# raulmur/ORB_SLAM2

Hardware: AMD Instinct MI355X
Metric: frames/s ORB extract+match, 1241x376 gray, 2000 kpts, 8 lvls (higher is better)
Workload: dtype u8

## Files before the change

### orb_slam2_amd/csrc/orbhip_api.hip

```cpp
#include <cstdarg>
#include <unistd.h>
#include <sys/syscall.h>
#include "orbhip_ctx.h"

static thread_local std::string g_err;
orbhip_status orbhip_set_error(orbhip_status st, const char* fmt, ...)
{
    char buf[512]; va_list ap; va_start(ap, fmt); vsnprintf(buf, sizeof buf, fmt, ap); va_end(ap);
    g_err = buf; return st;
}

static const char* kKernelNames[K_COUNT] = {"k_pyramid_level", "k_fast_cells", "k_blur", "k_quadtree", "k_describe",
                                            "k_match_grid", "k_match_candidates", "k_match_select", "k_undistort_keys", "k_remap"};

static const signed char kPatternHost[256 * 4] = {
#include "brief_pattern_31.inc"
};

void prof_collect(orbhip_ctx* c)
{
    for (auto& s : c->pending) {
        (void)hipEventSynchronize(s.b);
        float ms = 0; (void)hipEventElapsedTime(&ms, s.a, s.b);
        c->tot_ms[s.k] += ms; c->launches[s.k] += s.counts;
// ... 422 lines not shown
        std::vector<unsigned> mask(8 * 64, 0u);
        for (int q = 0; q < 8; q++) for (int l = 0; l < 64; l++) for (int b = 0; b < 4; b++) {
            const int r = 4 * q + (l >> 4), d = l & 15, v = r - 15, uu = 4 * d + b - 15;
            if (r <= 30 && d <= 7 && abs(uu) <= 15 && abs(uu) <= umax[abs(v)]) mask[q * 64 + l] |= 0xffu << (8 * b);
        }
        TRY(upload(&c->d_ic_mask, mask));
    }
    {
        const int psd = fc_pstride(c) / 4, nd = psd * std::max(c->fc_maxph, 1);
        c->fc_np = (nd + 63) / 64;
        const int np8 = (c->fc_np + 7) & ~7;
        std::vector<int4> tab((size_t)(np8 / 4) * 2 * 64);
        for (int k = 0; k < np8; k++) for (int l = 0; l < 64; l++) {
            const int pos = 64 * k + l, row = pos / psd, col4 = 4 * (pos % psd);
            int* r = &tab[(size_t)((k >> 2) * 2) * 64 + l].x; int* d = &tab[(size_t)((k >> 2) * 2 + 1) * 64 + l].x;
            r[k & 3] = row; d[k & 3] = col4;
        }
        TRY(upload(&c->d_fc_dma, tab));
    }
    TRY(dalloc(&c->d_pyr, B * c->plane_frame_bytes + 256)); TRY(dalloc(&c->d_blur, B * c->plane_frame_bytes + 256));
    TRY(dalloc(&c->d_cell_count, B * c->cells.size())); TRY(dalloc(&c->d_cell_cand, B * c->cand_slots_per_frame));
    TRY(dalloc(&c->d_qt_val, B * c->qt_per_frame)); TRY(dalloc(&c->d_qt_code, B * c->qt_per_frame)); TRY(dalloc(&c->d_qt_node, B * c->qt_per_frame));
    TRY(dalloc(&c->d_lvl_kp, B * c->lvl_kp_per_frame));
    for (int k = 0; k < 3; k++) {
        TRY(dalloc(&c->d_lvl_n[k], B * L));
        c->out_off_kp = (B * sizeof(int) + 255) & ~(size_t)255; c->out_off_desc = c->out_off_kp + ((B * c->out_cap * sizeof(orbhip_keypoint) + 255) & ~(size_t)255);
        c->out_block_bytes = c->out_off_desc + B * c->out_cap * 32;
        TRY(dalloc(&c->d_out_block[k], c->out_block_bytes));
        if (e == hipSuccess) { c->d_out_n[k] = reinterpret_cast<int*>(c->d_out_block[k]); c->d_out_kp[k] = reinterpret_cast<orbhip_keypoint*>(c->d_out_block[k] + c->out_off_kp); c->d_out_desc[k] = c->d_out_block[k] + c->out_off_desc; }
        if (e == hipSuccess) e = hipMemset(c->d_lvl_n[k], 0, B * L * sizeof(int));
        if (e == hipSuccess) e = hipMemset(c->d_out_n[k], 0, B * sizeof(int));
    }
    TRY(dalloc(&c->d_grid_start, B * (ORBHIP_GRID_CELLS + 1))); TRY(dalloc(&c->d_grid_items, B * c->out_cap)); TRY(dalloc(&c->d_grid_xy, B * c->out_cap));
    TRY(dalloc(&c->d_cand, B * c->lvl0_cap * (size_t)c->lvl0_cap)); TRY(dalloc(&c->d_ncand, B * c->lvl0_cap)); TRY(dalloc(&c->d_top, B * c->lvl0_cap * (size_t)5));
    TRY(dalloc(&c->d_prev, B * c->out_cap * 2)); TRY(dalloc(&c->d_m12, B * c->out_cap)); TRY(dalloc(&c->d_nm, B));
#undef TRY
    if (e != hipSuccess) { fail(ORBHIP_ERR_HIP, "device allocation failed: %s", hipGetErrorString(e)); orbhip_destroy(c); return ORBHIP_ERR_HIP; }
    *out = c;
    return ORBHIP_OK;
}

extern "C" int orbhip_keypoint_capacity(const orbhip_ctx* c) { return c ? c->out_cap : 0; }

extern "C" orbhip_status orbhip_get_scale_tables(const orbhip_ctx* c, float* sf, float* isf, float* s2, float* is2, int32_t* fpl)
{
    if (!c) return fail(ORBHIP_ERR_INVALID, "null context");
    for (int i = 0; i < c->L; i++) { if (sf) sf[i] = c->sf[i]; if (isf) isf[i] = c->isf[i]; if (s2) s2[i] = c->s2[i]; if (is2) is2[i] = c->is2[i]; if (fpl) fpl[i] = c->nfeat[i]; }
    return ORBHIP_OK;
}
extern "C" orbhip_status orbhip_level_size(const orbhip_ctx* c, int level, int* w, int* h)
{
    if (!c || level < 0 || level >= c->L) return fail(ORBHIP_ERR_INVALID, "bad level");
    if (w) *w = c->geom[level].w; if (h) *h = c->geom[level].h;
    return ORBHIP_OK;
}

extern "C" orbhip_status orbhip_set_blur_rounding(orbhip_ctx* c, int mode)
{
    if (!c || (mode != 0 && mode != 1)) return fail(ORBHIP_ERR_INVALID, "blur_round_mode is 0 (generic C++) or 1 (x86 SSE2 build)");
    c->cfg.blur_round_mode = mode;
    return ORBHIP_OK;
}

extern "C" orbhip_status orbhip_set_fp_contract(orbhip_ctx* c, int mode)
{
    if (!c || (mode != 0 && mode != 1)) return fail(ORBHIP_ERR_INVALID, "fp_contract is 0 (two roundings) or 1 (gcc's fused forms)");
    c->fp_contract = mode;
// ... 61 lines not shown
    HIPCHK(hipSetDevice(c->cfg.device));
    c->cur = (c->cur + 1) % 3;
    const int cur = c->cur;
    c->last_img0 = d_img0; c->last_img0_fstride = frame_stride; c->last_img0_pitch = row_stride; c->d_last_uright = nullptr; c->last_n_valid = false; c->fgrid_valid = false; c->rrows_valid = false;
    for (int k = 0; k < 3; k++) if (c->match_pending[k] && (k == (cur + 1) % 3)) { HIPCHK(hipStreamWaitEvent(c->stream, c->ev_match[k], 0)); c->match_pending[k] = false; }
    for (auto& hs : c->sets) if (hs.busy && hs.out_buf == cur && hs.nchunks > 0) HIPCHK(hipStreamWaitEvent(c->stream, hs.ev_d2h[hs.nchunks - 1], 0));
    return ORBHIP_OK;
}

orbhip_status run_pipeline(orbhip_ctx* c, int nimg, const uint8_t* d_img0, long long frame_stride, int row_stride,
                           int match_prev, int window, float nnratio, int check_ori)
{
    orbhip_status st = begin_batch(c, d_img0, frame_stride, row_stride); if (st != ORBHIP_OK) return st;
    const int cur = c->cur, prev = (cur + 2) % 3;
    const int ngroups = std::min((int)c->xstreams.size() + 1, nimg);
    ExtractParams P = make_params(c, d_img0, frame_stride, row_stride);
    if (ngroups > 1) { HIPCHK(hipEventRecord(c->ev_fork, c->stream)); }
    for (int gi = 0; gi < ngroups; gi++) {
        const int f0 = (int)((long long)nimg * gi / ngroups), f1 = (int)((long long)nimg * (gi + 1) / ngroups), nf = f1 - f0;
        hipStream_t s = gi == 0 ? c->stream : c->xstreams[gi - 1];
        if (gi > 0) HIPCHK(hipStreamWaitEvent(s, c->ev_fork, 0));
        if (nf <= 0) continue;
        st = pipeline_frames(c, P, f0, nf, s, ngroups == 1); if (st != ORBHIP_OK) return st;
        if (gi > 0) { HIPCHK(hipEventRecord(c->xevents[gi - 1], s)); HIPCHK(hipStreamWaitEvent(c->stream, c->xevents[gi - 1], 0)); }
    }
    if (match_prev) {
        MatchParams M; memset(&M, 0, sizeof M);
        M.kp1 = c->distorted ? c->d_out_kpun[prev] : c->d_out_kp[prev]; M.desc1 = c->d_out_desc[prev]; M.n1 = c->d_out_n[prev]; M.n1_lvl0 = c->d_lvl_n[prev];
        M.kp2 = c->distorted ? c->d_out_kpun[cur] : c->d_out_kp[cur]; M.desc2 = c->d_out_desc[cur]; M.n2 = c->d_out_n[cur];
        M.lvl_stride = c->L; M.list1 = nullptr; M.prev_from_kp1 = 1;
        M.cap = c->out_cap; M.min_x = c->bounds.min_x; M.min_y = c->bounds.min_y; M.max_x = c->bounds.max_x; M.max_y = c->bounds.max_y;
        M.grid_start = c->d_grid_start; M.grid_items = c->d_grid_items; M.grid_xy = c->d_grid_xy; M.cand = c->d_cand; M.top = c->d_top; M.ncand = c->d_ncand; M.cand_stride = c->lvl0_cap; M.lvl0_cap = c->lvl0_cap;
        M.prev = c->d_prev; M.matches12 = c->d_m12; M.nmatches = c->d_nm; M.window = window; M.nnratio = nnratio; M.check_ori = check_ori; M.slot0 = 0;
        if (orbhip_match_select_big(c->out_cap, c->lvl0_cap)) {
            if (!c->d_match_ws) HIPCHK(dalloc(&c->d_match_ws, (size_t)c->B * orbhip_match_select_ints(c->out_cap, c->lvl0_cap)));
            M.big_ws = c->d_match_ws;
        }
        hipStream_t ms = c->serial ? c->stream : c->mstream;
        HIPCHK(hipEventRecord(c->ev_extract, c->stream));
        HIPCHK(hipStreamWaitEvent(ms, c->ev_extract, 0));
        { ProfScope ps(c, K_MGRID, ms); orbhip_launch_match_grid(M, nimg, ms); }
        { ProfScope ps(c, K_MCAND, ms); orbhip_launch_match_candidates(M, nimg, ms); }
        { ProfScope ps(c, K_MSELECT, ms); orbhip_launch_match_select(M, nimg, ms); }
        HIPCHK(hipEventRecord(c->ev_match[cur], ms));
        c->match_pending[cur] = true;
    }
    c->last_matched = match_prev != 0;
    c->last_nimg = nimg;
    HIPCHK(hipGetLastError());
    return ORBHIP_OK;
}

extern "C" orbhip_status orbhip_extract_device(orbhip_ctx* c, int nimg, const uint8_t* d_imgs, size_t frame_stride, int row_stride,
                                               int match_prev, int window, float nnratio, int check_ori)
{
    if (!c || !d_imgs) return fail(ORBHIP_ERR_INVALID, "null argument");
    if (nimg < 1 || nimg > c->B) return fail(ORBHIP_ERR_INVALID, "nimg %d outside 1..%d", nimg, c->B);
    if (row_stride < c->cfg.width) return fail(ORBHIP_ERR_INVALID, "row stride %d < width %d", row_stride, c->cfg.width);
    c->last_from_host = false;
    return run_pipeline(c, nimg, d_imgs, (long long)frame_stride, row_stride, match_prev, window, nnratio, check_ori);
}

void orbhip_internal_outputs(orbhip_ctx* c, const uint8_t** d_desc, const int** d_n, int* cap, int* last_nimg, int* device, hipStream_t* s)
{
    *d_desc = c->d_out_desc[c->cur]; *d_n = c->d_out_n[c->cur]; *cap = c->out_cap; *last_nimg = c->last_nimg; *device = c->cfg.device; *s = c->stream;
}

extern "C" orbhip_status orbhip_sync(orbhip_ctx* c)
// ... 123 lines not shown
```

### orb_slam2_amd/csrc/orbhip_internal.h

```cpp
#pragma once
#include <hip/hip_runtime.h>
#include <cstdint>
#include "../../include/orbhip.h"

#include <cstdlib>
inline hipError_t orbhip_dmalloc(void** p, size_t bytes)
{
    const hipError_t e = hipMalloc(p, bytes);
    if (e != hipSuccess) return e;
    static const int poison = [] { const char* v = getenv("ORBHIP_POISON"); return v && *v ? atoi(v) & 255 : -1; }();
    if (poison < 0) return hipSuccess;
    const hipError_t m = hipMemset(*p, poison, bytes);
    return m != hipSuccess ? m : hipDeviceSynchronize();
}

#define ORBHIP_MAX_LEVELS 16
#define ORBHIP_QT_DEPTH 13
#define ORBHIP_GRID_COLS 64
#define ORBHIP_GRID_ROWS 48
#define ORBHIP_GRID_CELLS (ORBHIP_GRID_COLS * ORBHIP_GRID_ROWS)
#define ORBHIP_HISTO_LENGTH 30
#define ORBHIP_TH_LOW 50
#define ORBHIP_EDGE 16

// ... 40 lines not shown
    const int4* blur_band;
    const int2* xtab; const int2* ytab; const PyrGroup* xgrp;
    const unsigned* ic_mask;
    const float* patternf;
    int iniTh, minTh, blur_round_mode, fp_contract;
    int qt_maxn;
    int qt_maxcells;
    int qt_scr;
    int fc_pstride, fc_prows, fc_sstride, fc_srows, fc_listcap;
    int fc_cell0, fc_ncells;
    int fc_pbytes, fc_np; const int4* fc_dma;
    const short2* pc_xr; const short2* pc_yr; int pc_ntx, pc_nty, pc_buf0, pc_buf1, pc_xcap, pc_ycap;
};

struct MatchParams {
    const orbhip_keypoint* kp1; const uint8_t* desc1; const int* n1;
    const int* n1_lvl0; int lvl_stride;
    const int* list1;
    int prev_from_kp1;
    const orbhip_keypoint* kp2; const uint8_t* desc2; const int* n2;
    int cap;
    float min_x, min_y, max_x, max_y;
    int* grid_start; int* grid_items; float2* grid_xy;
    unsigned* cand; int* ncand; int cand_stride;
    unsigned* top;
    int lvl0_cap;
    float* prev;
    int* matches12; int* nmatches;
    int window; float nnratio; int check_ori;
    int slot0;
    int grid_all_levels;
    int* big_ws;
};
size_t orbhip_match_select_ints(int cap, int lvl0_cap);
bool orbhip_match_select_big(int cap, int lvl0_cap);

struct StereoSide {
    const orbhip_keypoint* kp; const uint8_t* desc; const int* n;
    const uint8_t* img0; long long img0_frame_stride; int img0_pitch;
    const uint8_t* pyr; long long plane_frame_bytes;
};
struct StereoParams {
    const LevelGeom* geom; StereoSide L, R;
    int cap, im_h;
    int* row_start; int* row_items; int row_cap;
    float* u_right; float* depth; int* sad;
    float mbf, maxD;
};
hipError_t orbhip_copy_async(void* dst, const void* src, size_t bytes, hipMemcpyKind kind, hipStream_t s);
int orbhip_device_numa_node(int device);
bool orbhip_bind_thread_to_node(int node);
void orbhip_launch_stereo(const StereoParams& T, int nslots, int max_left, hipStream_t s, bool rows_ready = false);
void orbhip_launch_stereo_rows(const StereoParams& T, int nslots, hipStream_t s);

struct ProjParams {
    const orbhip_keypoint* kp; const uint8_t* desc; const float* u_right; int n;
    float min_x, min_y, max_x, max_y;
    const int* grid_start; const int* grid_items; const float2* grid_xy;
    const orbhip_proj_query* q; const uint8_t* qdesc; int nq;
    const orbhip_map_point* pts; const orbhip_projection* proj; orbhip_proj_query* q_out;
    unsigned* cand; int* ncand; int cand_stride;
    unsigned* top;
    const unsigned char* blocked_in; unsigned char* blocked_out; int* feature_query; int* nmatches; int* events;
    int mode; float nnratio; int th_high, check_ori;
    int* big_ws;
};
bool orbhip_proj_select_big(int n);
void orbhip_launch_proj(const ProjParams& J, hipStream_t s, bool fp_contract = false);
// ... 121 lines not shown
```

### orb_slam2_amd/csrc/orbhip_kernels_match.hip

```cpp
#include "orbhip_internal.h"
#include <cstdlib>
#include <cstring>
#include <type_traits>

#define WAVE 64
#define IMAX 0x7fffffff

#define NN_T 256
#define NN_QPT 4
#define NN_ROWS 256
#define NN_CHUNK 8192

struct NNPart { int best, second; long long idx; };

__global__ __launch_bounds__(NN_T) void k_hamming_nn(const unsigned long long* q, int nq, const unsigned long long* db, long long ndb,
                                                     long long base, NNPart* parts, int nchunks)
{
    __shared__ unsigned long long s_db[NN_ROWS * 4];
    const int tid = threadIdx.x, chunk = blockIdx.y;
    const int q0 = (blockIdx.x * NN_T + tid) * NN_QPT;
    unsigned long long qa[NN_QPT][4];
    unsigned kb[NN_QPT], ks[NN_QPT];
#pragma unroll
    for (int k = 0; k < NN_QPT; k++) {
// ... 432 lines not shown
        const int a = c ? s_cnt[c - 1] : 0, b = s_cnt[c];
        for (int i = a + 1; i < b; i++) { const int v = gitems[i]; int j = i - 1; while (j >= a && gitems[j] > v) { gitems[j + 1] = gitems[j]; j--; } gitems[j + 1] = v; }
    }
    __threadfence_block();
    __syncthreads();
    for (int t = tid; t < total; t += 256) { const orbhip_keypoint k = kp[gitems[t]]; float2 xy; xy.x = k.x; xy.y = k.y; gxy[t] = xy; }
}

size_t orbhip_match_grid_lds(int cap) { return sizeof(int) * (ORBHIP_GRID_CELLS + 1 + (size_t)cap) + sizeof(unsigned short) * ((size_t)cap + 2); }

void orbhip_launch_match_grid(const MatchParams& M, int nslots, hipStream_t s)
{
    const float gwInv = (float)ORBHIP_GRID_COLS / (float)(M.max_x - M.min_x), ghInv = (float)ORBHIP_GRID_ROWS / (float)(M.max_y - M.min_y);
    size_t lds_max = (size_t)150 * 1024;
#ifdef ORBHIP_TEST_HOOKS
    if (const char* e = getenv("ORBHIP_TEST_MATCH_GRID_LDS_MAX")) lds_max = (size_t)atol(e);
#endif
    if (orbhip_match_grid_lds(M.cap) <= lds_max) hipLaunchKernelGGL(k_match_grid, dim3(nslots, 1, 1), dim3(256, 1, 1), orbhip_match_grid_lds(M.cap), s, M, gwInv, ghInv);
    else hipLaunchKernelGGL(k_match_grid_big, dim3(nslots, 1, 1), dim3(256, 1, 1), 0, s, M, gwInv, ghInv);
}

__device__ __forceinline__ int wave_min_dpp(int v)
{
    v = min(v, __builtin_amdgcn_update_dpp(IMAX, v, 0x111, 0xf, 0xf, false));
    v = min(v, __builtin_amdgcn_update_dpp(IMAX, v, 0x112, 0xf, 0xf, false));
    v = min(v, __builtin_amdgcn_update_dpp(IMAX, v, 0x114, 0xf, 0xe, false));
    v = min(v, __builtin_amdgcn_update_dpp(IMAX, v, 0x118, 0xf, 0xc, false));
    v = min(v, __builtin_amdgcn_update_dpp(IMAX, v, 0x142, 0xa, 0xf, false));
    v = min(v, __builtin_amdgcn_update_dpp(IMAX, v, 0x143, 0xc, 0xf, false));
    return __builtin_amdgcn_readlane(v, 63);
}

#define MS_K 4
#define MS_REC (MS_K + 1)
#define MS_NONE 0xFFFFFFFFu
#define MC_CHUNKS 8
__global__ __launch_bounds__(256) void k_match_candidates(MatchParams M, float gwInv, float ghInv)
{
    const int wave = __builtin_amdgcn_readfirstlane(threadIdx.x >> 6), lane = threadIdx.x & 63, slot = blockIdx.y + M.slot0;
    const int j1 = blockIdx.x * 4 + wave;
    const int n1l = M.n1_lvl0[slot * M.lvl_stride];
    if (j1 >= n1l || j1 >= M.lvl0_cap) return;
    const int i1 = M.list1 ? M.list1[(long long)slot * M.lvl0_cap + j1] : j1;
    const int nitems = M.grid_start[(long long)slot * (ORBHIP_GRID_CELLS + 1) + ORBHIP_GRID_CELLS];
    const int* gitems = M.grid_items + (long long)slot * M.cap;
    const float2* gxy = M.grid_xy + (long long)slot * M.cap;
    unsigned* cand = M.cand + ((long long)slot * M.lvl0_cap + j1) * M.cand_stride;
    const orbhip_keypoint* kp1 = M.kp1 + (long long)slot * M.cap;
    const float x = M.prev_from_kp1 ? kp1[i1].x : M.prev[((long long)slot * M.cap + i1) * 2];
    const float y = M.prev_from_kp1 ? kp1[i1].y : M.prev[((long long)slot * M.cap + i1) * 2 + 1];
    const float r = (float)M.window;
    const unsigned long long* d1 = (const unsigned long long*)(M.desc1 + ((long long)slot * M.cap + i1) * 32);
    const unsigned long long q0 = d1[0], q1 = d1[1], q2 = d1[2], q3 = d1[3];
    const unsigned long long below = (1ull << lane) - 1ull;
    int nc = 0;
    int tk[MS_K]; unsigned te[MS_K]; int nsel = 0;
#pragma unroll
    for (int k = 0; k < MS_K; k++) { tk[k] = IMAX; te[k] = MS_NONE; }
    const int* gstart = M.grid_start + (long long)slot * (ORBHIP_GRID_CELLS + 1);
    const float cl = __fmul_rn(__fsub_rn(__fsub_rn(x, M.min_x), r), gwInv), ch = __fmul_rn(__fadd_rn(__fsub_rn(x, M.min_x), r), gwInv);
    const int col_lo = cl >= 1.0f ? (int)fminf(floorf(cl) - 1.0f, (float)ORBHIP_GRID_COLS) : 0;
    const int col_hi = ch < (float)(ORBHIP_GRID_COLS - 2) ? (int)fmaxf(ceilf(ch) + 2.0f, 0.0f) : ORBHIP_GRID_COLS;
    const int t_lo = __builtin_amdgcn_readfirstlane(gstart[min(col_lo, col_hi) * ORBHIP_GRID_ROWS]), t_hi = __builtin_amdgcn_readfirstlane(gstart[col_hi * ORBHIP_GRID_ROWS]);
    (void)nitems;
    for (int tb = t_lo; tb < t_hi; tb += 64 * MC_CHUNKS) {
        float2 k[MC_CHUNKS]; int it[MC_CHUNKS];
#pragma unroll
        for (int c = 0; c < MC_CHUNKS; c++) {
            const int t = tb + 64 * c + lane;
            k[c].x = 0.0f; k[c].y = 0.0f; it[c] = 0;
            if (t < t_hi) { k[c] = gxy[t]; it[c] = gitems[t]; }
        }
#pragma unroll
        for (int c = 0; c < MC_CHUNKS; c++) {
            if (tb + 64 * c >= t_hi) break;
            const bool ok = tb + 64 * c + lane < t_hi && fabsf(__fsub_rn(k[c].x, x)) < r && fabsf(__fsub_rn(k[c].y, y)) < r;
            const unsigned long long m = __ballot(ok);
            if (m == 0) continue;
            const int pos = nc + __popcll(m & below);
            if (ok && pos < M.cand_stride) {
                const unsigned long long* d2 = (const unsigned long long*)(M.desc2 + ((long long)slot * M.cap + it[c]) * 32);
                const int dist = __popcll(q0 ^ d2[0]) + __popcll(q1 ^ d2[1]) + __popcll(q2 ^ d2[2]) + __popcll(q3 ^ d2[3]);
                unsigned rec = (unsigned)it[c] | ((unsigned)dist << 20);
                cand[pos] = rec;
                int key = (dist << 20) | pos;
                nsel++;
#pragma unroll
                for (int k = 0; k < MS_K; k++) if (key < tk[k]) { const int tkk = tk[k]; const unsigned tee = te[k]; tk[k] = key; te[k] = rec; key = tkk; rec = tee; }
            }
            nc += __popcll(m);
        }
    }
    nc = min(nc, M.cand_stride);
    if (lane == 0) M.ncand[(long long)slot * M.lvl0_cap + j1] = nc;
    unsigned out = MS_NONE; int popped = 0;
#pragma unroll
    for (int r = 0; r < MS_K; r++) {
        const int m = wave_min_dpp(tk[0]);
        if (m == IMAX) break;
        const int owner = __ffsll((long long)__ballot(tk[0] == m)) - 1;
        const unsigned rec = (unsigned)__builtin_amdgcn_readlane((int)te[0], owner);
        if (lane == r) out = rec;
        if (lane == owner) {
            popped++;
#pragma unroll
            for (int k = 0; k + 1 < MS_K; k++) { tk[k] = tk[k + 1]; te[k] = te[k + 1]; }
            tk[MS_K - 1] = IMAX; te[MS_K - 1] = MS_NONE;
        }
    }
    const bool more = __ballot(nsel > popped) != 0ull;
    unsigned* top = M.top + ((long long)slot * M.lvl0_cap + j1) * MS_REC;
    if (lane < MS_K) top[lane] = out;
    if (lane == MS_K) top[MS_K] = more ? 1u : 0u;
}

void orbhip_launch_match_candidates(const MatchParams& M, int nslots, hipStream_t s)
{
    const float gwInv = (float)ORBHIP_GRID_COLS / (float)(M.max_x - M.min_x), ghInv = (float)ORBHIP_GRID_ROWS / (float)(M.max_y - M.min_y);
    hipLaunchKernelGGL(k_match_candidates, dim3((M.lvl0_cap + 3) / 4, nslots, 1), dim3(256, 1, 1), 0, s, M, gwInv, ghInv);
}


#define MS_T 256

__device__ __forceinline__ int orbhip_match_select_ints_d(int cap, int lvl0_cap) { return 4 * cap + 4 * lvl0_cap + ORBHIP_HISTO_LENGTH + 8; }
template <bool BIG> __device__ __forceinline__ void match_select_body(const MatchParams& M)
{
    typedef typename std::conditional<BIG, volatile int, int>::type TI;
    typedef typename std::conditional<BIG, volatile float, float>::type TF;
    const int slot = blockIdx.x + M.slot0, tid = threadIdx.x, lane = tid & 63, wave = tid >> 6;
    const int n1 = M.n1[slot], n2 = M.n2[slot];
    const int n1l = min(M.n1_lvl0[slot * M.lvl_stride], M.lvl0_cap);
    const int* list1 = M.list1 ? M.list1 + (long long)slot * M.lvl0_cap : nullptr;
    HIP_DYNAMIC_SHARED(int, lds)
    TI* s_md = BIG ? M.big_ws + (long long)(blockIdx.x + M.slot0) * (long long)orbhip_match_select_ints_d(M.cap, M.lvl0_cap) : lds;
    TI* s_m21 = s_md + M.cap;
    TI* s_m12 = s_m21 + M.cap;
    TI* s_bin = s_m12 + M.lvl0_cap;
    TI* s_nc = s_bin + M.lvl0_cap;
    TI* s_hist = s_nc + M.lvl0_cap;
    TI* s_stamp = s_hist + ORBHIP_HISTO_LENGTH + 8;
    TF* s_ang1 = reinterpret_cast<TF*>(s_stamp + M.cap);
    TF* s_ang2 = s_ang1 + M.lvl0_cap;
    auto amin = [](TI* p, int v) { atomicMin(const_cast<int*>(p), v); };
    auto aadd = [](TI* p, int v) { atomicAdd(const_cast<int*>(p), v); };
    const orbhip_keypoint* kp1 = M.kp1 + (long long)slot * M.cap;
    const orbhip_keypoint* kp2 = M.kp2 + (long long)slot * M.cap;
    int* m12 = M.matches12 + (long long)slot * M.cap;
    float* prev = M.prev + (long long)slot * M.cap * 2;
    const unsigned* cand0 = M.cand + (long long)slot * M.lvl0_cap * M.cand_stride;
    for (int i = tid; i < n2; i += MS_T) { s_md[i] = IMAX; s_m21[i] = -1; s_stamp[i] = IMAX; s_ang2[i] = kp2[i].angle; }
    for (int i = tid; i < n1l; i += MS_T) { s_m12[i] = -1; s_bin[i] = -1; s_nc[i] = M.ncand[(long long)slot * M.lvl0_cap + i]; s_ang1[i] = kp1[list1 ? list1[i] : i].angle; }
    for (int i = tid; i < ORBHIP_HISTO_LENGTH + 8; i += MS_T) s_hist[i] = 0;
    for (int i = tid; i < n1; i += MS_T) { m12[i] = -1; if (M.prev_from_kp1) { prev[2 * i] = kp1[i].x; prev[2 * i + 1] = kp1[i].y; } }
    __syncthreads();
    if (wave == 0) {
        const float factor = 1.0f / ORBHIP_HISTO_LENGTH;
        const unsigned* top0 = M.top + (long long)slot * M.lvl0_cap * MS_REC;
        auto rot_bin = [&](int j1, int i2) -> int {
            float rot = __fsub_rn(s_ang1[j1], s_ang2[i2]);
            if (rot < 0.0f) rot = __fadd_rn(rot, 360.0f);
            int bin = (int)roundf(__fmul_rn(rot, factor));
            if (bin == ORBHIP_HISTO_LENGTH) bin = 0;
            return min(max(bin, 0), ORBHIP_HISTO_LENGTH - 1);
        };
        for (int jb = 0; jb < n1l; jb += 64) {
            const int j1 = jb + lane;
            const bool inb = j1 < n1l;
            int ei[MS_K], ed[MS_K]; int nk = 0;
#pragma unroll
            for (int k = 0; k < MS_K; k++) {
                const unsigned t = (inb && s_nc[j1] != 0) ? top0[(long long)j1 * MS_REC + k] : MS_NONE;
                ei[k] = (int)(t & 0xFFFFFu); ed[k] = (int)((t >> 20) & 0x1FFu);
                if (t != MS_NONE) nk = k + 1;
            }
            const bool more = nk > 0 && top0[(long long)j1 * MS_REC + MS_K] != 0u;
            int stamped = -1;
            unsigned long long todo = __ballot(nk > 0);
            while (todo) {
                const bool mine = (todo >> lane) & 1ull;
                const int lowest = __ffsll((long long)todo) - 1;
                int a = -1, b = -1;
#pragma unroll
                for (int k = 0; k < MS_K; k++)
                    if (mine && k < nk && b < 0 && !(s_md[ei[k]] <= ed[k])) { if (a < 0) a = k; else b = k; }
                const int ia = a >= 0 ? ei[a] : 0, da = a >= 0 ? ed[a] : IMAX, db = b >= 0 ? ed[b] : IMAX;
                const bool exhausted = mine && more && b < 0;
                const bool accept = mine && !exhausted && a >= 0 && da <= ORBHIP_TH_LOW && (float)da < __fmul_rn((float)db, M.nnratio);
                const int want = accept ? ia : -1;
                if (stamped >= 0 && stamped != want && s_stamp[stamped] == j1) s_stamp[stamped] = IMAX;
                __builtin_amdgcn_wave_barrier();
                if (want >= 0) amin(&s_stamp[want], j1);
                stamped = want;
                __builtin_amdgcn_wave_barrier();
                bool unsure = false;
                const int last = b >= 0 ? b : nk - 1;
#pragma unroll
                for (int k = 0; k < MS_K; k++)
                    if (mine && lane != lowest && k <= last && !(s_md[ei[k]] <= ed[k]) && s_stamp[ei[k]] < j1) unsure = true;
                const unsigned long long bad = __ballot(unsure || exhausted);
                const int first_bad = bad ? __ffsll((long long)bad) - 1 : 64;
                const unsigned long long commit = first_bad == 64 ? todo : (todo & ((1ull << first_bad) - 1ull));
                const bool win = ((commit >> lane) & 1ull) && accept;
                if (win) {
                    const int old = s_m21[ia];
                    if (old >= 0) s_m12[old] = -1;
                    s_m12[j1] = ia; s_m21[ia] = j1; s_md[ia] = da;
                    if (s_stamp[ia] == j1) s_stamp[ia] = IMAX;
                    stamped = -1;
                    if (M.check_ori) { const int bin = rot_bin(j1, ia); s_bin[j1] = bin; aadd(&s_hist[bin], 1); }
                }
                __builtin_amdgcn_wave_barrier();
                todo &= ~commit;
                if (first_bad == 64) break;
                if (first_bad != lowest || !((__ballot(exhausted) >> first_bad) & 1ull)) continue;
                todo &= ~(1ull << first_bad);
                if (lane == first_bad && stamped >= 0 && s_stamp[stamped] == j1) s_stamp[stamped] = IMAX;
                const int js = jb + first_bad, nc = s_nc[js];
                const unsigned* cand = cand0 + (long long)js * M.cand_stride;
                int best = IMAX, second = IMAX, bidx = -1;
                for (int cb = 0; cb < nc; cb += 64) {
                    const int t = cb + lane;
                    const unsigned e = t < nc ? cand[t] : 0u;
                    const int i2 = (int)(e & 0xFFFFFu), dist = (int)(e >> 20);
                    const bool valid = t < nc && !(s_md[i2] <= dist);
                    const int key = valid ? ((dist << 6) | lane) : IMAX;
                    const int k1 = wave_min_dpp(key);
                    if (k1 == IMAX) continue;
                    const int first = k1 & 63, wmin = k1 >> 6, ci = __builtin_amdgcn_readlane(i2, first);
                    const int k2 = wave_min_dpp(lane == first ? IMAX : key);
                    const int wsec = k2 == IMAX ? IMAX : (k2 >> 6);
                    if (wmin < best) { second = min(best, wsec); best = wmin; bidx = ci; } else second = min(second, wmin);
                }
                if (best <= ORBHIP_TH_LOW && (float)best < __fmul_rn((float)second, M.nnratio)) {
                    if (lane == 0) {
                        const int old = s_m21[bidx];
                        if (old >= 0) s_m12[old] = -1;
                        s_m12[js] = bidx; s_m21[bidx] = js; s_md[bidx] = best;
                        if (M.check_ori) { const int bin = rot_bin(js, bidx); s_bin[js] = bin; s_hist[bin] = s_hist[bin] + 1; }
                    }
                }
                __builtin_amdgcn_wave_barrier();
            }
        }
    }
    if (wave != 0) return;
    __builtin_amdgcn_wave_barrier();
    if (M.check_ori) {
        if (lane == 0) {
            int max1 = 0, max2 = 0, max3 = 0, ind1 = -1, ind2 = -1, ind3 = -1;
            for (int i = 0; i < ORBHIP_HISTO_LENGTH; i++) {
                const int s = s_hist[i];
                if (s > max1) { max3 = max2; max2 = max1; max1 = s; ind3 = ind2; ind2 = ind1; ind1 = i; }
                else if (s > max2) { max3 = max2; max2 = s; ind3 = ind2; ind2 = i; }
                else if (s > max3) { max3 = s; ind3 = i; }
            }
            if ((float)max2 < __fmul_rn(0.1f, (float)max1)) { ind2 = -1; ind3 = -1; }
            else if ((float)max3 < __fmul_rn(0.1f, (float)max1)) { ind3 = -1; }
            s_hist[ORBHIP_HISTO_LENGTH] = ind1; s_hist[ORBHIP_HISTO_LENGTH + 1] = ind2; s_hist[ORBHIP_HISTO_LENGTH + 2] = ind3;
        }
        __builtin_amdgcn_wave_barrier();
        const int ind1 = s_hist[ORBHIP_HISTO_LENGTH], ind2 = s_hist[ORBHIP_HISTO_LENGTH + 1], ind3 = s_hist[ORBHIP_HISTO_LENGTH + 2];
        for (int j = lane; j < n1l; j += 64) { const int b = s_bin[j]; if (b >= 0 && b != ind1 && b != ind2 && b != ind3) s_m12[j] = -1; }
        __builtin_amdgcn_wave_barrier();
    }
    int cnt = 0;
    for (int j = lane; j < n1l; j += 64) {
        const int m = s_m12[j];
        if (m >= 0) { const int i1 = list1 ? list1[j] : j; cnt++; m12[i1] = m; prev[2 * i1] = kp2[m].x; prev[2 * i1 + 1] = kp2[m].y; }
    }
#pragma unroll
    for (int off = 32; off >= 1; off >>= 1) cnt += __shfl_xor(cnt, off);
    if (lane == 0) M.nmatches[slot] = cnt;
}

__global__ __launch_bounds__(MS_T) void k_match_select(MatchParams M) { match_select_body<false>(M); }
__global__ __launch_bounds__(MS_T) void k_match_select_big(MatchParams M) { match_select_body<true>(M); }

#define MS_LDS_BUDGET (158 * 1024)
size_t orbhip_match_select_ints(int cap, int lvl0_cap) { return (size_t)4 * cap + (size_t)4 * lvl0_cap + ORBHIP_HISTO_LENGTH + 8; }
bool orbhip_match_select_big(int cap, int lvl0_cap)
{
    const char* env = getenv("ORBHIP_SELECT_BIG");
    const bool force = env && env[0] == '1';
    return force || sizeof(int) * orbhip_match_select_ints(cap, lvl0_cap) > MS_LDS_BUDGET;
}
void orbhip_launch_match_select(const MatchParams& M, int nslots, hipStream_t s)
{
    if (M.big_ws) hipLaunchKernelGGL(k_match_select_big, dim3(nslots, 1, 1), dim3(MS_T, 1, 1), 0, s, M);
    else hipLaunchKernelGGL(k_match_select, dim3(nslots, 1, 1), dim3(MS_T, 1, 1), sizeof(int) * orbhip_match_select_ints(M.cap, M.lvl0_cap), s, M);
}
```

### orb_slam2_amd/csrc/orbhip_search.hip

```cpp
#include "orbhip_ctx.h"

template <typename Layout, typename Launch> static hipError_t arena_call(int device, hipStream_t s, Layout layout, Launch launch, size_t floor = 0)
{
    hipError_t e = arena_layout(device, layout, floor);
    if (e == hipSuccess) e = arena_upload(s);
    if (e == hipSuccess) { launch(); e = hipGetLastError(); }
    if (e == hipSuccess) e = arena_download(s);
    if (e != hipSuccess) (void)hipStreamSynchronize(s);
    return e;
}

static thread_local struct HeldSlots { int device = -1; size_t floor = 0; std::vector<BestParams> B; std::vector<int> live_of_slot; } g_held;

void launch_feature_grid(const orbhip_keypoint* kp, const int* d_n, int cap, const orbhip_bounds& b, int* grid_start, int* grid_items, float2* grid_xy,
                         int nslots, int slot0, hipStream_t s)
{
    MatchParams M; memset(&M, 0, sizeof M);
    M.kp2 = kp; M.n2 = d_n; M.cap = cap; M.min_x = b.min_x; M.min_y = b.min_y; M.max_x = b.max_x; M.max_y = b.max_y;
    M.grid_start = grid_start; M.grid_items = grid_items; M.grid_xy = grid_xy; M.grid_all_levels = 1; M.slot0 = slot0;
    orbhip_launch_match_grid(M, nslots, s);
}

static bool projection_ok(const orbhip_projection* P)
{
// ... 473 lines not shown
    if (e == hipSuccess) e = hipMemcpy(best_dist, dbd, (size_t)nq * 4, hipMemcpyDeviceToHost);
    if (e == hipSuccess) e = hipMemcpy(second_dist, dsd, (size_t)nq * 4, hipMemcpyDeviceToHost);
    if (e != hipSuccess) st = fail(ORBHIP_ERR_HIP, "hamming_nn: %s", hipGetErrorString(e));
    (void)hipFree(dq); (void)hipFree(ddb); (void)hipFree(dbi); (void)hipFree(dbd); (void)hipFree(dsd);
    return st;
}

extern "C" orbhip_status orbhip_search_for_initialization_bounds(int device, const orbhip_keypoint* kps1, const uint8_t* desc1, int n1,
                                                          const orbhip_keypoint* kps2, const uint8_t* desc2, int n2, const orbhip_bounds* bounds,
                                                          float* prev_matched, int32_t* matches12, int window, float nnratio, int check_ori, int* nmatches)
{
    OrbApiTimer api_timer;
    if (n1 < 0 || n2 < 0 || !nmatches || (n1 > 0 && (!kps1 || !desc1 || !prev_matched || !matches12)) || (n2 > 0 && (!kps2 || !desc2)) || !bounds || !(bounds->max_x > bounds->min_x) || !(bounds->max_y > bounds->min_y))
        return fail(ORBHIP_ERR_INVALID, "bad argument");
    *nmatches = 0;
    for (int i = 0; i < n1; i++) matches12[i] = -1;
    if (n1 == 0) return ORBHIP_OK;
    if (!device_present()) return fail(ORBHIP_ERR_HIP, "no HIP device available: no CPU fallback");
    HIPCHK(hipSetDevice(device));
    hipStream_t ts = orbhip_thread_stream(device);
    std::vector<int> list1; for (int i = 0; i < n1; i++) if (kps1[i].octave <= 0) list1.push_back(i);
    int n2l0 = 0; for (int i = 0; i < n2; i++) n2l0 += kps2[i].octave == 0;
    const int cap = std::max(std::max(n1, n2), 1), l0cap = std::max((int)list1.size(), 1), cstride = std::max(n2l0, 1);
    orbhip_keypoint *dk1 = nullptr, *dk2 = nullptr; uint8_t *dd1 = nullptr, *dd2 = nullptr; int *dn = nullptr, *dlist = nullptr, *dgs = nullptr, *dgi = nullptr, *dnc = nullptr, *dm12 = nullptr, *dbig = nullptr; float2* dgxy = nullptr;
    unsigned* dcand = nullptr; unsigned* dtop = nullptr; float* dprev = nullptr;
    const int hn[4] = {n1, n2, (int)list1.size(), 0}; int hres[4] = {0, 0, 0, 0};
    const hipError_t e = arena_call(device, ts, [&](Arena& A) {
        A.io(&dk1, cap, kps1, n1); A.io(&dk2, cap, kps2, n2); A.io(&dd1, (size_t)cap * 32, desc1, (size_t)n1 * 32); A.io(&dd2, (size_t)cap * 32, desc2, (size_t)n2 * 32);
        A.io(&dlist, l0cap, (const int*)list1.data(), list1.size());
        A.io(&dn, 8, hn, 4, hres, 4);
        A.io(&dprev, (size_t)cap * 2, (const float*)prev_matched, (size_t)n1 * 2, prev_matched, (size_t)n1 * 2);
        A.io(&dm12, cap, (const int*)nullptr, 0, matches12, n1);
        A.take(&dgs, ORBHIP_GRID_CELLS + 1); A.take(&dgi, cap); A.take(&dgxy, cap); A.take(&dnc, l0cap);
        A.take(&dcand, (size_t)l0cap * cstride); A.take(&dtop, (size_t)l0cap * 5);
        if (orbhip_match_select_big(cap, l0cap)) A.take(&dbig, orbhip_match_select_ints(cap, l0cap));
    }, [&] {
        MatchParams M; memset(&M, 0, sizeof M);
        M.kp1 = dk1; M.desc1 = dd1; M.n1 = dn; M.n1_lvl0 = dn + 2; M.kp2 = dk2; M.desc2 = dd2; M.n2 = dn + 1; M.lvl_stride = 0; M.list1 = dlist; M.prev_from_kp1 = 0;
        M.cap = cap; M.min_x = bounds->min_x; M.min_y = bounds->min_y; M.max_x = bounds->max_x; M.max_y = bounds->max_y; M.grid_start = dgs; M.grid_items = dgi; M.grid_xy = dgxy; M.cand = dcand; M.top = dtop; M.ncand = dnc; M.cand_stride = cstride; M.lvl0_cap = l0cap;
        M.prev = dprev; M.matches12 = dm12; M.nmatches = dn + 3; M.window = window; M.nnratio = nnratio; M.check_ori = check_ori; M.big_ws = dbig;
        orbhip_launch_match_grid(M, 1, ts); orbhip_launch_match_candidates(M, 1, ts); orbhip_launch_match_select(M, 1, ts);
    });
    if (e != hipSuccess) return fail(ORBHIP_ERR_HIP, "search_for_initialization: %s", hipGetErrorString(e));
    *nmatches = hres[3];
    return ORBHIP_OK;
}

static bool whole_image(int im_w, int im_h, orbhip_bounds* b) { if (im_w < 1 || im_h < 1) return false; b->min_x = 0.0f; b->min_y = 0.0f; b->max_x = (float)im_w; b->max_y = (float)im_h; return true; }
extern "C" orbhip_status orbhip_search_by_projection(int device, const orbhip_keypoint* kps, const uint8_t* desc, const float* u_right, const uint8_t* blocked, int n,
                                                     int im_w, int im_h, const orbhip_proj_query* queries, const uint8_t* query_desc, int nq,
                                                     int mode, float nnratio, int th_high, int check_ori, int32_t* feature_query, int* nmatches)
{
    orbhip_bounds b; if (!whole_image(im_w, im_h, &b)) return fail(ORBHIP_ERR_INVALID, "bad argument");
    return orbhip_search_by_projection_bounds(device, kps, desc, u_right, blocked, n, &b, queries, query_desc, nq, mode, nnratio, th_high, check_ori, feature_query, nmatches);
}
extern "C" orbhip_status orbhip_search_best_in_window(int device, const orbhip_keypoint* kps, const uint8_t* desc, const float* u_right, int n, int im_w, int im_h,
                                                      const float* inv_level_sigma2, int nlevels, const orbhip_best_query* queries, const uint8_t* query_desc, int nq,
                                                      int chi2_gate, int32_t* best_idx, int32_t* best_dist)
{
    orbhip_bounds b; if (!whole_image(im_w, im_h, &b)) return fail(ORBHIP_ERR_INVALID, "bad argument");
    return orbhip_search_best_in_window_bounds(device, kps, desc, u_right, n, &b, inv_level_sigma2, nlevels, queries, query_desc, nq, chi2_gate, best_idx, best_dist);
}
extern "C" orbhip_status orbhip_search_for_initialization(int device, const orbhip_keypoint* kps1, const uint8_t* desc1, int n1,
                                                          const orbhip_keypoint* kps2, const uint8_t* desc2, int n2, int im_w, int im_h,
                                                          float* prev_matched, int32_t* matches12, int window, float nnratio, int check_ori, int* nmatches)
{
    orbhip_bounds b; if (!whole_image(im_w, im_h, &b)) return fail(ORBHIP_ERR_INVALID, "bad argument");
    return orbhip_search_for_initialization_bounds(device, kps1, desc1, n1, kps2, desc2, n2, &b, prev_matched, matches12, window, nnratio, check_ori, nmatches);
// ... 49 lines not shown
```

Before: 204,900.

## Compact match-select state into grid-item index space and pack top-k records

The candidate and top-k records now store grid-item indices instead of frame-2 keypoint indices. The per-frame-2 arrays in match select are sized by grid items rather than out_cap, and distance plus owner are merged into one packed word. The 'more' flag moves into the high bit of the last top record, so each record is four words and can be loaded with a single uint4. The top-k table is also staged into LDS, and the orientation bin is packed into m12, which removes the bin, nc and m21 arrays. The aim is a smaller LDS footprint that avoids the slow global-memory 'big' path, and fewer scattered loads. The cost is an extra gitems indirection and tighter bit-packing limits.

Result: no change. 205,400 (median of 3 runs) (+0.2%).

```diff
diff --git a/orb_slam2_amd/csrc/orbhip_api.hip b/orb_slam2_amd/csrc/orbhip_api.hip
--- a/orb_slam2_amd/csrc/orbhip_api.hip
+++ b/orb_slam2_amd/csrc/orbhip_api.hip
@@ -478,7 +478,7 @@
         if (e == hipSuccess) e = hipMemset(c->d_out_n[k], 0, B * sizeof(int));
     }
     TRY(dalloc(&c->d_grid_start, B * (ORBHIP_GRID_CELLS + 1))); TRY(dalloc(&c->d_grid_items, B * c->out_cap)); TRY(dalloc(&c->d_grid_xy, B * c->out_cap));
-    TRY(dalloc(&c->d_cand, B * c->lvl0_cap * (size_t)c->lvl0_cap)); TRY(dalloc(&c->d_ncand, B * c->lvl0_cap)); TRY(dalloc(&c->d_top, B * c->lvl0_cap * (size_t)5));
+    TRY(dalloc(&c->d_cand, B * c->lvl0_cap * (size_t)c->lvl0_cap)); TRY(dalloc(&c->d_ncand, B * c->lvl0_cap)); TRY(dalloc(&c->d_top, B * c->lvl0_cap * (size_t)4));
     TRY(dalloc(&c->d_prev, B * c->out_cap * 2)); TRY(dalloc(&c->d_m12, B * c->out_cap)); TRY(dalloc(&c->d_nm, B));
 #undef TRY
     if (e != hipSuccess) { fail(ORBHIP_ERR_HIP, "device allocation failed: %s", hipGetErrorString(e)); orbhip_destroy(c); return ORBHIP_ERR_HIP; }
@@ -606,8 +606,8 @@
         M.cap = c->out_cap; M.min_x = c->bounds.min_x; M.min_y = c->bounds.min_y; M.max_x = c->bounds.max_x; M.max_y = c->bounds.max_y;
         M.grid_start = c->d_grid_start; M.grid_items = c->d_grid_items; M.grid_xy = c->d_grid_xy; M.cand = c->d_cand; M.top = c->d_top; M.ncand = c->d_ncand; M.cand_stride = c->lvl0_cap; M.lvl0_cap = c->lvl0_cap;
         M.prev = c->d_prev; M.matches12 = c->d_m12; M.nmatches = c->d_nm; M.window = window; M.nnratio = nnratio; M.check_ori = check_ori; M.slot0 = 0;
-        if (orbhip_match_select_big(c->out_cap, c->lvl0_cap)) {
-            if (!c->d_match_ws) HIPCHK(dalloc(&c->d_match_ws, (size_t)c->B * orbhip_match_select_ints(c->out_cap, c->lvl0_cap)));
+        if (orbhip_match_select_big(c->lvl0_cap, c->lvl0_cap)) {
+            if (!c->d_match_ws) HIPCHK(dalloc(&c->d_match_ws, (size_t)c->B * orbhip_match_select_ints(c->lvl0_cap, c->lvl0_cap)));
             M.big_ws = c->d_match_ws;
         }
         hipStream_t ms = c->serial ? c->stream : c->mstream;
diff --git a/orb_slam2_amd/csrc/orbhip_internal.h b/orb_slam2_amd/csrc/orbhip_internal.h
--- a/orb_slam2_amd/csrc/orbhip_internal.h
+++ b/orb_slam2_amd/csrc/orbhip_internal.h
@@ -96,8 +96,8 @@
     int grid_all_levels;
     int* big_ws;
 };
-size_t orbhip_match_select_ints(int cap, int lvl0_cap);
-bool orbhip_match_select_big(int cap, int lvl0_cap);
+size_t orbhip_match_select_ints(int lvl0_cap, int f2_cap);
+bool orbhip_match_select_big(int lvl0_cap, int f2_cap);
 
 struct StereoSide {
     const orbhip_keypoint* kp; const uint8_t* desc; const int* n;
diff --git a/orb_slam2_amd/csrc/orbhip_kernels_match.hip b/orb_slam2_amd/csrc/orbhip_kernels_match.hip
--- a/orb_slam2_amd/csrc/orbhip_kernels_match.hip
+++ b/orb_slam2_amd/csrc/orbhip_kernels_match.hip
@@ -488,7 +488,8 @@
 }
 
 #define MS_K 4
-#define MS_REC (MS_K + 1)
+#define MS_REC MS_K
+#define MS_MORE 0x80000000u
 #define MS_NONE 0xFFFFFFFFu
 #define MC_CHUNKS 8
 __global__ __launch_bounds__(256) void k_match_candidates(MatchParams M, float gwInv, float ghInv)
@@ -537,7 +538,7 @@
             if (ok && pos < M.cand_stride) {
                 const unsigned long long* d2 = (const unsigned long long*)(M.desc2 + ((long long)slot * M.cap + it[c]) * 32);
                 const int dist = __popcll(q0 ^ d2[0]) + __popcll(q1 ^ d2[1]) + __popcll(q2 ^ d2[2]) + __popcll(q3 ^ d2[3]);
-                unsigned rec = (unsigned)it[c] | ((unsigned)dist << 20);
+                unsigned rec = (unsigned)(tb + 64 * c + lane) | ((unsigned)dist << 20);
                 cand[pos] = rec;
                 int key = (dist << 20) | pos;
                 nsel++;
@@ -566,8 +567,7 @@
     }
     const bool more = __ballot(nsel > popped) != 0ull;
     unsigned* top = M.top + ((long long)slot * M.lvl0_cap + j1) * MS_REC;
-    if (lane < MS_K) top[lane] = out;
-    if (lane == MS_K) top[MS_K] = more ? 1u : 0u;
+    if (lane < MS_K) top[lane] = (lane == MS_K - 1 && more) ? (out | MS_MORE) : out;
 }
 
 void orbhip_launch_match_candidates(const MatchParams& M, int nslots, hipStream_t s)
@@ -579,58 +579,70 @@
 
 #define MS_T 256
 
-__device__ __forceinline__ int orbhip_match_select_ints_d(int cap, int lvl0_cap) { return 4 * cap + 4 * lvl0_cap + ORBHIP_HISTO_LENGTH + 8; }
+__device__ __forceinline__ int orbhip_match_select_ints_d(int lvl0_cap, int f2_cap) { return 3 * f2_cap + 2 * lvl0_cap + ORBHIP_HISTO_LENGTH + 8; }
 template <bool BIG> __device__ __forceinline__ void match_select_body(const MatchParams& M)
 {
     typedef typename std::conditional<BIG, volatile int, int>::type TI;
     typedef typename std::conditional<BIG, volatile float, float>::type TF;
     const int slot = blockIdx.x + M.slot0, tid = threadIdx.x, lane = tid & 63, wave = tid >> 6;
-    const int n1 = M.n1[slot], n2 = M.n2[slot];
+    const int n1 = M.n1[slot];
     const int n1l = min(M.n1_lvl0[slot * M.lvl_stride], M.lvl0_cap);
+    const int nitems = min(M.grid_start[(long long)slot * (ORBHIP_GRID_CELLS + 1) + ORBHIP_GRID_CELLS], M.cand_stride);
     const int* list1 = M.list1 ? M.list1 + (long long)slot * M.lvl0_cap : nullptr;
+    const int* gitems = M.grid_items + (long long)slot * M.cap;
+    const unsigned* top0 = M.top + (long long)slot * M.lvl0_cap * MS_REC;
     HIP_DYNAMIC_SHARED(int, lds)
-    TI* s_md = BIG ? M.big_ws + (long long)(blockIdx.x + M.slot0) * (long long)orbhip_match_select_ints_d(M.cap, M.lvl0_cap) : lds;
-    TI* s_m21 = s_md + M.cap;
-    TI* s_m12 = s_m21 + M.cap;
-    TI* s_bin = s_m12 + M.lvl0_cap;
-    TI* s_nc = s_bin + M.lvl0_cap;
-    TI* s_hist = s_nc + M.lvl0_cap;
-    TI* s_stamp = s_hist + ORBHIP_HISTO_LENGTH + 8;
-    TF* s_ang1 = reinterpret_cast<TF*>(s_stamp + M.cap);
-    TF* s_ang2 = s_ang1 + M.lvl0_cap;
+    const unsigned* s_top = BIG ? top0 : reinterpret_cast<const unsigned*>(lds);
+    TI* s_f2 = BIG ? M.big_ws + (long long)slot * (long long)orbhip_match_select_ints_d(M.lvl0_cap, M.cand_stride) : lds + MS_REC * M.lvl0_cap;
+    TI* s_stamp = s_f2 + M.cand_stride;
+    TF* s_ang2 = reinterpret_cast<TF*>(s_stamp + M.cand_stride);
+    TI* s_m12 = reinterpret_cast<TI*>(s_ang2 + M.cand_stride);
+    TF* s_ang1 = reinterpret_cast<TF*>(s_m12 + M.lvl0_cap);
+    TI* s_hist = reinterpret_cast<TI*>(s_ang1 + M.lvl0_cap);
     auto amin = [](TI* p, int v) { atomicMin(const_cast<int*>(p), v); };
     auto aadd = [](TI* p, int v) { atomicAdd(const_cast<int*>(p), v); };
+    auto md = [&](int t) -> int { return (int)((unsigned)s_f2[t] >> 20); };
     const orbhip_keypoint* kp1 = M.kp1 + (long long)slot * M.cap;
     const orbhip_keypoint* kp2 = M.kp2 + (long long)slot * M.cap;
     int* m12 = M.matches12 + (long long)slot * M.cap;
     float* prev = M.prev + (long long)slot * M.cap * 2;
     const unsigned* cand0 = M.cand + (long long)slot * M.lvl0_cap * M.cand_stride;
-    for (int i = tid; i < n2; i += MS_T) { s_md[i] = IMAX; s_m21[i] = -1; s_stamp[i] = IMAX; s_ang2[i] = kp2[i].angle; }
-    for (int i = tid; i < n1l; i += MS_T) { s_m12[i] = -1; s_bin[i] = -1; s_nc[i] = M.ncand[(long long)slot * M.lvl0_cap + i]; s_ang1[i] = kp1[list1 ? list1[i] : i].angle; }
+    if (!BIG) for (int i = tid; i < MS_REC * n1l; i += MS_T) lds[i] = (int)top0[i];
+    for (int i = tid; i < nitems; i += MS_T) { s_f2[i] = -1; s_stamp[i] = IMAX; s_ang2[i] = kp2[gitems[i]].angle; }
+    for (int i = tid; i < n1l; i += MS_T) { s_m12[i] = -1; s_ang1[i] = kp1[list1 ? list1[i] : i].angle; }
     for (int i = tid; i < ORBHIP_HISTO_LENGTH + 8; i += MS_T) s_hist[i] = 0;
     for (int i = tid; i < n1; i += MS_T) { m12[i] = -1; if (M.prev_from_kp1) { prev[2 * i] = kp1[i].x; prev[2 * i + 1] = kp1[i].y; } }
     __syncthreads();
-    if (wave == 0) {
+    if (wave != 0) return;
+    {
         const float factor = 1.0f / ORBHIP_HISTO_LENGTH;
-        const unsigned* top0 = M.top + (long long)slot * M.lvl0_cap * MS_REC;
-        auto rot_bin = [&](int j1, int i2) -> int {
-            float rot = __fsub_rn(s_ang1[j1], s_ang2[i2]);
+        auto rot_bin = [&](int j1, int t2) -> int {
+            float rot = __fsub_rn(s_ang1[j1], s_ang2[t2]);
             if (rot < 0.0f) rot = __fadd_rn(rot, 360.0f);
             int bin = (int)roundf(__fmul_rn(rot, factor));
             if (bin == ORBHIP_HISTO_LENGTH) bin = 0;
             return min(max(bin, 0), ORBHIP_HISTO_LENGTH - 1);
         };
+        auto accept_match = [&](int j1, int t, int d, bool atomic_hist) {
+            const int old = s_f2[t];
+            if (old != -1) s_m12[old & 0xFFFFF] = -1;
+            int w = t;
+            if (M.check_ori) { const int bin = rot_bin(j1, t); w |= bin << 20; if (atomic_hist) aadd(&s_hist[bin], 1); else s_hist[bin] = s_hist[bin] + 1; }
+            s_m12[j1] = w; s_f2[t] = (d << 20) | j1;
+        };
         for (int jb = 0; jb < n1l; jb += 64) {
             const int j1 = jb + lane;
             const bool inb = j1 < n1l;
+            uint4 tr; tr.x = MS_NONE; tr.y = MS_NONE; tr.z = MS_NONE; tr.w = MS_NONE;
+            if (inb) tr = *reinterpret_cast<const uint4*>(s_top + (long long)j1 * MS_REC);
+            const unsigned tw[MS_K] = {tr.x, tr.y, tr.z, tr.w};
             int ei[MS_K], ed[MS_K]; int nk = 0;
 #pragma unroll
             for (int k = 0; k < MS_K; k++) {
-                const unsigned t = (inb && s_nc[j1] != 0) ? top0[(long long)j1 * MS_REC + k] : MS_NONE;
-                ei[k] = (int)(t & 0xFFFFFu); ed[k] = (int)((t >> 20) & 0x1FFu);
-                if (t != MS_NONE) nk = k + 1;
+                ei[k] = (int)(tw[k] & 0xFFFFFu); ed[k] = (int)((tw[k] >> 20) & 0x1FFu);
+                if (tw[k] != MS_NONE) nk = k + 1;
             }
-            const bool more = nk > 0 && top0[(long long)j1 * MS_REC + MS_K] != 0u;
+            const bool more = tr.w != MS_NONE && (tr.w & MS_MORE) != 0u;
             int stamped = -1;
             unsigned long long todo = __ballot(nk > 0);
             while (todo) {
@@ -639,7 +651,7 @@
                 int a = -1, b = -1;
 #pragma unroll
                 for (int k = 0; k < MS_K; k++)
-                    if (mine && k < nk && b < 0 && !(s_md[ei[k]] <= ed[k])) { if (a < 0) a = k; else b = k; }
+                    if (mine && k < nk && b < 0 && !(md(ei[k]) <= ed[k])) { if (a < 0) a = k; else b = k; }
                 const int ia = a >= 0 ? ei[a] : 0, da = a >= 0 ? ed[a] : IMAX, db = b >= 0 ? ed[b] : IMAX;
                 const bool exhausted = mine && more && b < 0;
                 const bool accept = mine && !exhausted && a >= 0 && da <= ORBHIP_TH_LOW && (float)da < __fmul_rn((float)db, M.nnratio);
@@ -653,18 +665,15 @@
                 const int last = b >= 0 ? b : nk - 1;
 #pragma unroll
                 for (int k = 0; k < MS_K; k++)
-                    if (mine && lane != lowest && k <= last && !(s_md[ei[k]] <= ed[k]) && s_stamp[ei[k]] < j1) unsure = true;
+                    if (mine && lane != lowest && k <= last && !(md(ei[k]) <= ed[k]) && s_stamp[ei[k]] < j1) unsure = true;
                 const unsigned long long bad = __ballot(unsure || exhausted);
                 const int first_bad = bad ? __ffsll((long long)bad) - 1 : 64;
                 const unsigned long long commit = first_bad == 64 ? todo : (todo & ((1ull << first_bad) - 1ull));
                 const bool win = ((commit >> lane) & 1ull) && accept;
                 if (win) {
-                    const int old = s_m21[ia];
-                    if (old >= 0) s_m12[old] = -1;
-                    s_m12[j1] = ia; s_m21[ia] = j1; s_md[ia] = da;
+                    accept_match(j1, ia, da, true);
                     if (s_stamp[ia] == j1) s_stamp[ia] = IMAX;
                     stamped = -1;
-                    if (M.check_ori) { const int bin = rot_bin(j1, ia); s_bin[j1] = bin; aadd(&s_hist[bin], 1); }
                 }
                 __builtin_amdgcn_wave_barrier();
                 todo &= ~commit;
@@ -672,35 +681,29 @@
                 if (first_bad != lowest || !((__ballot(exhausted) >> first_bad) & 1ull)) continue;
                 todo &= ~(1ull << first_bad);
                 if (lane == first_bad && stamped >= 0 && s_stamp[stamped] == j1) s_stamp[stamped] = IMAX;
-                const int js = jb + first_bad, nc = s_nc[js];
+                const int js = jb + first_bad, nc = M.ncand[(long long)slot * M.lvl0_cap + js];
                 const unsigned* cand = cand0 + (long long)js * M.cand_stride;
                 int best = IMAX, second = IMAX, bidx = -1;
                 for (int cb = 0; cb < nc; cb += 64) {
                     const int t = cb + lane;
                     const unsigned e = t < nc ? cand[t] : 0u;
-                    const int i2 = (int)(e & 0xFFFFFu), dist = (int)(e >> 20);
-                    const bool valid = t < nc && !(s_md[i2] <= dist);
+                    const int t2 = (int)(e & 0xFFFFFu), dist = (int)(e >> 20);
+                    const bool valid = t < nc && !(md(t2) <= dist);
                     const int key = valid ? ((dist << 6) | lane) : IMAX;
                     const int k1 = wave_min_dpp(key);
                     if (k1 == IMAX) continue;
-                    const int first = k1 & 63, wmin = k1 >> 6, ci = __builtin_amdgcn_readlane(i2, first);
+                    const int first = k1 & 63, wmin = k1 >> 6, ci = __builtin_amdgcn_readlane(t2, first);
                     const int k2 = wave_min_dpp(lane == first ? IMAX : key);
                     const int wsec = k2 == IMAX ? IMAX : (k2 >> 6);
                     if (wmin < best) { second = min(best, wsec); best = wmin; bidx = ci; } else second = min(second, wmin);
                 }
                 if (best <= ORBHIP_TH_LOW && (float)best < __fmul_rn((float)second, M.nnratio)) {
-                    if (lane == 0) {
-                        const int old = s_m21[bidx];
-                        if (old >= 0) s_m12[old] = -1;
-                        s_m12[js] = bidx; s_m21[bidx] = js; s_md[bidx] = best;
-                        if (M.check_ori) { const int bin = rot_bin(js, bidx); s_bin[js] = bin; s_hist[bin] = s_hist[bin] + 1; }
-                    }
+                    if (lane == 0) accept_match(js, bidx, best, false);
                 }
                 __builtin_amdgcn_wave_barrier();
             }
         }
     }
-    if (wave != 0) return;
     __builtin_amdgcn_wave_barrier();
     if (M.check_ori) {
         if (lane == 0) {
@@ -717,13 +720,13 @@
         }
         __builtin_amdgcn_wave_barrier();
         const int ind1 = s_hist[ORBHIP_HISTO_LENGTH], ind2 = s_hist[ORBHIP_HISTO_LENGTH + 1], ind3 = s_hist[ORBHIP_HISTO_LENGTH + 2];
-        for (int j = lane; j < n1l; j += 64) { const int b = s_bin[j]; if (b >= 0 && b != ind1 && b != ind2 && b != ind3) s_m12[j] = -1; }
+        for (int j = lane; j < n1l; j += 64) { const int w = s_m12[j]; if (w >= 0) { const int b = w >> 20; if (b != ind1 && b != ind2 && b != ind3) s_m12[j] = -1; } }
         __builtin_amdgcn_wave_barrier();
     }
     int cnt = 0;
     for (int j = lane; j < n1l; j += 64) {
-        const int m = s_m12[j];
-        if (m >= 0) { const int i1 = list1 ? list1[j] : j; cnt++; m12[i1] = m; prev[2 * i1] = kp2[m].x; prev[2 * i1 + 1] = kp2[m].y; }
+        const int w = s_m12[j];
+        if (w >= 0) { const int i1 = list1 ? list1[j] : j, m = gitems[w & 0xFFFFF]; cnt++; m12[i1] = m; prev[2 * i1] = kp2[m].x; prev[2 * i1 + 1] = kp2[m].y; }
     }
 #pragma unroll
     for (int off = 32; off >= 1; off >>= 1) cnt += __shfl_xor(cnt, off);
@@ -734,15 +737,16 @@
 __global__ __launch_bounds__(MS_T) void k_match_select_big(MatchParams M) { match_select_body<true>(M); }
 
 #define MS_LDS_BUDGET (158 * 1024)
-size_t orbhip_match_select_ints(int cap, int lvl0_cap) { return (size_t)4 * cap + (size_t)4 * lvl0_cap + ORBHIP_HISTO_LENGTH + 8; }
-bool orbhip_match_select_big(int cap, int lvl0_cap)
+size_t orbhip_match_select_ints(int lvl0_cap, int f2_cap) { return (size_t)3 * f2_cap + (size_t)2 * lvl0_cap + ORBHIP_HISTO_LENGTH + 8; }
+static size_t match_select_lds(int lvl0_cap, int f2_cap) { return sizeof(int) * (orbhip_match_select_ints(lvl0_cap, f2_cap) + (size_t)MS_REC * lvl0_cap); }
+bool orbhip_match_select_big(int lvl0_cap, int f2_cap)
 {
     const char* env = getenv("ORBHIP_SELECT_BIG");
     const bool force = env && env[0] == '1';
-    return force || sizeof(int) * orbhip_match_select_ints(cap, lvl0_cap) > MS_LDS_BUDGET;
+    return force || match_select_lds(lvl0_cap, f2_cap) > MS_LDS_BUDGET;
 }
 void orbhip_launch_match_select(const MatchParams& M, int nslots, hipStream_t s)
 {
     if (M.big_ws) hipLaunchKernelGGL(k_match_select_big, dim3(nslots, 1, 1), dim3(MS_T, 1, 1), 0, s, M);
-    else hipLaunchKernelGGL(k_match_select, dim3(nslots, 1, 1), dim3(MS_T, 1, 1), sizeof(int) * orbhip_match_select_ints(M.cap, M.lvl0_cap), s, M);
-}
+    else hipLaunchKernelGGL(k_match_select, dim3(nslots, 1, 1), dim3(MS_T, 1, 1), match_select_lds(M.lvl0_cap, M.cand_stride), s, M);
+}
diff --git a/orb_slam2_amd/csrc/orbhip_search.hip b/orb_slam2_amd/csrc/orbhip_search.hip
--- a/orb_slam2_amd/csrc/orbhip_search.hip
+++ b/orb_slam2_amd/csrc/orbhip_search.hip
@@ -529,8 +529,8 @@
         A.io(&dprev, (size_t)cap * 2, (const float*)prev_matched, (size_t)n1 * 2, prev_matched, (size_t)n1 * 2);
         A.io(&dm12, cap, (const int*)nullptr, 0, matches12, n1);
         A.take(&dgs, ORBHIP_GRID_CELLS + 1); A.take(&dgi, cap); A.take(&dgxy, cap); A.take(&dnc, l0cap);
-        A.take(&dcand, (size_t)l0cap * cstride); A.take(&dtop, (size_t)l0cap * 5);
-        if (orbhip_match_select_big(cap, l0cap)) A.take(&dbig, orbhip_match_select_ints(cap, l0cap));
+        A.take(&dcand, (size_t)l0cap * cstride); A.take(&dtop, (size_t)l0cap * 4);
+        if (orbhip_match_select_big(l0cap, cstride)) A.take(&dbig, orbhip_match_select_ints(l0cap, cstride));
     }, [&] {
         MatchParams M; memset(&M, 0, sizeof M);
         M.kp1 = dk1; M.desc1 = dd1; M.n1 = dn; M.n1_lvl0 = dn + 2; M.kp2 = dk2; M.desc2 = dd2; M.n2 = dn + 1; M.lvl_stride = 0; M.list1 = dlist; M.prev_from_kp1 = 0;
```
